# ORNL/HydraGNN

Hardware: NVIDIA H100
Metric: atoms_per_sec_training_step (higher is better)
Workload: dtype tf32

## Files before the change

### hydragnn_b200/csrc/hgb_painn_tc.cu

```cuda
#include "hgb_tc.cuh"

namespace {

enum { UPD_FWD, UPD_POST, UPD_BWD_A, UPD_BWD };

constexpr int UF = 64;
constexpr int UPD_TILE = 64;
constexpr uint32_t UPD_STAGE = UPD_TILE * UF * 4;
constexpr uint32_t UPD_B = 2 * UF * UF * 4;
constexpr uint32_t UPD_G = UPD_TILE * 2 * UF * 4;
constexpr int UPD_THREADS = 160;
constexpr int upd_stages(int mode) { return mode == UPD_BWD ? 5 : 4; }

struct UpdParams {
  int n;
  const float* wuv;
  const float* buv;
  const float* s;
  const float* a;
  const float* gs_out;
  const float* gv_out;
  const float* g_mlp_in;
  const float* mlp_in;
  float* mlp_in_out;
  float* inner_out;
  float* s_out;
  float* v_out;
  float* ga;
  float* g_uv;
  float* gs;
  float* gv;
};

constexpr size_t upd_smem(int mode) {
  return 1024 + (mode == UPD_BWD ? 2 : 1) * (size_t)UPD_B + upd_stages(mode) * (size_t)UPD_STAGE + (mode == UPD_BWD ? (size_t)UPD_G : 0) +
         2 * upd_stages(mode) * 8 + 2 * UF * 4;
}

__device__ __forceinline__ void frag_ld(float* x, const float* p, int64_t ld, int node, int n) {
#pragma unroll
  for (int h = 0; h < 2; ++h) {
    const bool in = node + 8 * h < n;
    const float* r = p + (int64_t)(node + 8 * h) * ld;
#pragma unroll
    for (int i = 0; i < 8; ++i) {
      const float2 t = in ? __ldg(reinterpret_cast<const float2*>(r + 8 * i)) : make_float2(0.f, 0.f);
      x[4 * i + 2 * h] = t.x;
      x[4 * i + 2 * h + 1] = t.y;
    }
  }
}
__device__ __forceinline__ void frag_st(float* p, int64_t ld, int node, int n, const float* x) {
#pragma unroll
  for (int h = 0; h < 2; ++h)
    if (node + 8 * h < n) {
      float* r = p + (int64_t)(node + 8 * h) * ld;
#pragma unroll
      for (int i = 0; i < 8; ++i) *reinterpret_cast<float2*>(r + 8 * i) = make_float2(x[4 * i + 2 * h], x[4 * i + 2 * h + 1]);
    }
}

__device__ __forceinline__ void prefetch_rows_l2(const float* base, int64_t ld, int row0, int rows, int col0, int cols) {
  if (cols == ld) {
    asm volatile("cp.async.bulk.prefetch.L2.global [%0], %1;" ::"l"(base + (int64_t)row0 * ld), "r"((uint32_t)(rows * ld * 4)) : "memory");
    return;
  }
  for (int r = 0; r < rows; ++r)
    asm volatile("cp.async.bulk.prefetch.L2.global [%0], %1;" ::"l"(base + (int64_t)(row0 + r) * ld + col0), "r"((uint32_t)(cols * 4))
                 : "memory");
}

}

template <int MODE, bool LAST>
__global__ void __launch_bounds__(UPD_THREADS, 1) painn_update_tc_kernel(const __grid_constant__ CUtensorMap tmap_v, const UpdParams p) {
  constexpr int NA = LAST ? 2 : 3;
  constexpr bool BWD = MODE == UPD_BWD;
  constexpr int S = upd_stages(MODE);
  extern __shared__ uint8_t smem_raw[];
  uint8_t* smem = reinterpret_cast<uint8_t*>((reinterpret_cast<uintptr_t>(smem_raw) + 1023) & ~(uintptr_t)1023);
  uint8_t* sB = smem;
  uint8_t* sBd = sB + UPD_B;
  uint8_t* sA = sBd + (BWD ? UPD_B : 0);
  uint8_t* sG = sA + S * UPD_STAGE;
  uint64_t* full = reinterpret_cast<uint64_t*>(sG + (BWD ? UPD_G : 0));
  uint64_t* empty = full + S;
  float* sbias = reinterpret_cast<float*>(empty + S);

  const int warp = threadIdx.x >> 5, lane = threadIdx.x & 31;
  const int ntiles = (p.n + UPD_TILE - 1) / UPD_TILE;
  for (int i = threadIdx.x; i < 2 * UF; i += blockDim.x) sbias[i] = __ldg(p.buv + i);
  if (threadIdx.x == 0) {
    for (int s = 0; s < S; ++s) { mbar_init(full + s, 1); mbar_init(empty + s, 4); }
    fence_barrier_init();
  }
  __syncthreads();

  if (warp == 4) {
    if (lane == 0) {
      uint32_t it = 0;
      for (int t = blockIdx.x; t < ntiles; t += gridDim.x) {
        const int row0 = t * UPD_TILE, rows = min(UPD_TILE, p.n - row0);
        if (MODE == UPD_FWD || MODE == UPD_POST) prefetch_rows_l2(p.s, UF, row0, rows, 0, UF);
        if (MODE == UPD_POST) prefetch_rows_l2(p.a, NA * UF, row0, rows, 0, NA * UF);
        if (MODE == UPD_BWD_A || BWD) prefetch_rows_l2(p.gs_out, UF, row0, rows, 0, UF);
        if ((MODE == UPD_BWD_A || BWD) && !LAST) prefetch_rows_l2(p.gv_out, 3 * UF, row0, rows, 0, 3 * UF);
        if (BWD) {
          prefetch_rows_l2(p.g_mlp_in, 2 * UF, row0, rows, 0, 2 * UF);
          prefetch_rows_l2(p.mlp_in, 2 * UF, row0, rows, 0, UF);
          prefetch_rows_l2(p.a, NA * UF, row0, rows, 0, (NA - 1) * UF);
        }
        for (int d = 0; d < 3; ++d, ++it) {
          const int s = it % S;
          mbar_wait(empty + s, ((it / S) & 1) ^ 1);
          mbar_expect_tx(full + s, UPD_STAGE);
          tma_load_3d(sA + (size_t)s * UPD_STAGE, &tmap_v, full + s, 0, d, t * UPD_TILE);
          tma_load_3d(sA + (size_t)s * UPD_STAGE + UPD_STAGE / 2, &tmap_v, full + s, 32, d, t * UPD_TILE);
        }
      }
    }
    return;
  }

  for (int i = threadIdx.x; i < 2 * UF * UF; i += 128) {
    const float w = __ldg(p.wuv + i);
    const int r = i / UF, c = i % UF;
    *reinterpret_cast<float*>(sB + kmajor_sw128_off(r, c, 2 * UF)) = w;
    if (BWD) *reinterpret_cast<float*>(sBd + kmajor_sw128_off(c, r, UF)) = w;
  }
  fence_proxy_async();
  named_bar_sync(1, 128);

  const int wq = warp;
  const int rsub = wq * 16 + (lane >> 2);
  const int c2 = 2 * (lane & 3);
  const uint32_t sA_addr = smem_u32(sA), sB_addr = smem_u32(sB), sBd_addr = smem_u32(sBd);
  const uint32_t sG_addr = smem_u32(sG);

  float acc[64];
  uint32_t it = 0;
  for (int t = blockIdx.x; t < ntiles; t += gridDim.x) {
    const int node = t * UPD_TILE + rsub;
    float x0[32], x1[32], x2[32];
    if (MODE == UPD_FWD) {
      frag_ld(x0, p.s + c2, UF, node, p.n);
      frag_st(p.mlp_in_out + UF + c2, 2 * UF, node, p.n, x0);
    }
    if ((MODE == UPD_POST || MODE == UPD_BWD) && !LAST) frag_ld(x2, p.a + c2, NA * UF, node, p.n);
    if (BWD) {
      float g[32], q[32];
      frag_ld(g, p.gs_out + c2, UF, node, p.n);
      frag_ld(q, p.g_mlp_in + UF + c2, 2 * UF, node, p.n);
#pragma unroll
      for (int j = 0; j < 32; ++j) q[j] = g[j] + q[j];
      frag_st(p.gs + c2, UF, node, p.n, q);
      frag_ld(x0, p.a + (NA - 2) * UF + c2, NA * UF, node, p.n);
#pragma unroll
      for (int j = 0; j < 32; ++j) x0[j] = g[j] * x0[j];
      frag_ld(x1, p.mlp_in + c2, 2 * UF, node, p.n);
      frag_ld(q, p.g_mlp_in + c2, 2 * UF, node, p.n);
#pragma unroll
      for (int j = 0; j < 32; ++j) {
        const float nrm = x1[j];
        x1[j] = nrm > 0.f ? q[j] / nrm : 0.f;
      }
    }
#pragma unroll 1
    for (int d = 0; d < 3; ++d, ++it) {
      const int s = it % S;
      float gvo[32];
// ... 68 lines not shown
          const int r = rsub + 8 * ((j >> 1) & 1), col = 8 * (j >> 2) + c2 + (j & 1);
          vo[j] = *reinterpret_cast<const float*>(st + kmajor_sw128_off(r, col, UPD_TILE)) + x2[j] * acc[j];
        }
        __syncwarp();
        if (lane == 0) mbar_arrive(empty + s);
        frag_st(p.v_out + d * UF + c2, 3 * UF, node, p.n, vo);
      }
      if (BWD) {
#pragma unroll
        for (int j = 0; j < 32; ++j) {
          const float u = acc[j], w = acc[32 + j];
          const float g_vo = LAST ? 0.f : gvo[j], a_vv = LAST ? 0.f : x2[j];
          acc[j] = fmaf(x0[j], w, g_vo * a_vv);
          acc[32 + j] = fmaf(x0[j], u, x1[j] * w);
        }
        frag_st(p.g_uv + d * 2 * UF + c2, 3 * 2 * UF, node, p.n, acc);
        frag_st(p.g_uv + d * 2 * UF + UF + c2, 3 * 2 * UF, node, p.n, acc + 32);
        named_bar_sync(1, 128);
#pragma unroll
        for (int j = 0; j < 32; j += 2) {
          const int r = rsub + 8 * ((j >> 1) & 1), col = 8 * (j >> 2) + c2;
          *reinterpret_cast<float2*>(sG + kmajor_sw128_off(r, col, UPD_TILE)) = make_float2(acc[j], acc[j + 1]);
          *reinterpret_cast<float2*>(sG + kmajor_sw128_off(r, UF + col, UPD_TILE)) = make_float2(acc[32 + j], acc[33 + j]);
        }
        fence_proxy_async();
        named_bar_sync(1, 128);
        float dg[32];
#pragma unroll
        for (int j = 0; j < 32; ++j) dg[j] = 0.f;
        fence_regs<32>(dg);
        wgmma_fence();
#pragma unroll
        for (int kb = 0; kb < 4; ++kb)
#pragma unroll
          for (int k4 = 0; k4 < 4; ++k4)
            wgmma_tf32<2>(dg, make_desc(sG_addr + kb * (UPD_G / 4) + k4 * 32), make_desc(sBd_addr + kb * UF * 128 + k4 * 32));
        wgmma_commit();
        wgmma_wait<0>();
        fence_regs<32>(dg);
#pragma unroll
        for (int j = 0; j < 32; ++j) {
          float y = dg[j] + 0.f;
          if (!LAST) y += gvo[j];
          dg[j] = y;
        }
        frag_st(p.gv + d * UF + c2, 3 * UF, node, p.n, dg);
      }
    }
    if (MODE == UPD_POST) {
      float sv[32], ss[32];
      frag_ld(x1, p.s + c2, UF, node, p.n);
      frag_ld(sv, p.a + (NA - 2) * UF + c2, NA * UF, node, p.n);
      frag_ld(ss, p.a + (NA - 1) * UF + c2, NA * UF, node, p.n);
#pragma unroll
      for (int j = 0; j < 32; ++j) x1[j] = x1[j] + sv[j] * x0[j] + ss[j];
      frag_st(p.s_out + c2, UF, node, p.n, x1);
    }
    if (MODE == UPD_BWD_A) {
      float g[32];
      frag_ld(g, p.gs_out + c2, UF, node, p.n);
      if (!LAST) frag_st(p.ga + c2, NA * UF, node, p.n, x1);
#pragma unroll
// ... 15 lines not shown
}
__global__ void painn_update_tc_bwd_a_last_kernel(const float* __restrict__ gs_out, const float* __restrict__ inner, int64_t nf,
                                                  float* __restrict__ ga) {
  for (int64_t t = (int64_t)blockIdx.x * blockDim.x + threadIdx.x; t < nf; t += (int64_t)gridDim.x * blockDim.x) {
    const int64_t i = t / UF;
    const int c = (int)(t % UF);
    const float g = gs_out[t];
    ga[i * 2 * UF + c] = g * inner[t];
    ga[i * 2 * UF + UF + c] = g;
  }
}

namespace {

template <int MODE, bool LAST>
int launch_update(const float* v, const UpdParams& p, hgb_stream_t stream, const char* name) {
  CUtensorMap tm;
  const cuuint64_t dims[3] = {(cuuint64_t)UF, 3, (cuuint64_t)p.n};
  const cuuint64_t strides[2] = {(cuuint64_t)UF * 4, (cuuint64_t)3 * UF * 4};
  const cuuint32_t box[3] = {32, 1, (cuuint32_t)UPD_TILE};
  int rc = encode_tmap(&tm, v, 3, dims, strides, box, CU_TENSOR_MAP_SWIZZLE_128B);
  if (rc) return rc;
  constexpr size_t smem = upd_smem(MODE);
  static_assert(smem <= SMEM_MAX, "painn_update_tc: shared memory budget");
  static int per_sm = 0;
  if (!per_sm) {
    cudaFuncSetAttribute(painn_update_tc_kernel<MODE, LAST>, cudaFuncAttributeMaxDynamicSharedMemorySize, (int)smem);
    if (cudaOccupancyMaxActiveBlocksPerMultiprocessor(&per_sm, painn_update_tc_kernel<MODE, LAST>, UPD_THREADS, smem) != cudaSuccess ||
        per_sm < 1)
      per_sm = 1;
  }
  const int ntiles = (p.n + UPD_TILE - 1) / UPD_TILE;
  const int grid = ntiles < per_sm * HGB_NUM_SMS ? ntiles : per_sm * HGB_NUM_SMS;
  painn_update_tc_kernel<MODE, LAST><<<grid, UPD_THREADS, smem, (cudaStream_t)stream>>>(tm, p);
  HGB_LAUNCH_CHECK(name);
  return HGB_OK;
}

bool al16(const void* q) { return ((uintptr_t)q & 15) == 0; }

UpdParams upd_params(int n, const float* wuv, const float* buv) {
  UpdParams p = {};
  p.n = n;
  p.wuv = wuv;
  p.buv = buv;
  return p;
}

}

// ... 36 lines not shown
  if (last) {
    const int64_t nf = (int64_t)n * UF;
    painn_update_tc_bwd_a_last_kernel<<<hgb_grid_for(nf, 256), 256, 0, (cudaStream_t)stream>>>(gs_out, inner, nf, ga);
    HGB_LAUNCH_CHECK("painn_update_tc_bwd_a_last");
    return HGB_OK;
  }
  UpdParams p = upd_params(n, wuv, buv);
  p.gs_out = gs_out;
  p.gv_out = gv_out;
  p.ga = ga;
  return launch_update<UPD_BWD_A, false>(v, p, stream, "painn_update_tc_bwd_a");
}

extern "C" int hgb_painn_update_tc_bwd(const float* v, const float* gs_out, const float* gv_out, const float* g_mlp_in, const float* a,
                                       const float* mlp_in, const float* wuv, const float* buv, int32_t n, int32_t last, float* g_uv,
                                       float* gs, float* gv, hgb_stream_t stream) {
  HGB_REQUIRE(n >= 0 && v && gs_out && g_mlp_in && a && mlp_in && wuv && buv && g_uv && gs && gv && (last || gv_out),
              "painn_update_tc_bwd: bad arguments");
  HGB_REQUIRE(al16(v) && al16(gs_out) && al16(g_mlp_in) && al16(a) && al16(mlp_in) && al16(g_uv) && al16(gs) && al16(gv) &&
                  (last || al16(gv_out)),
              "painn_update_tc_bwd: operands must be 16-byte aligned");
  if (n == 0) return HGB_OK;
  UpdParams p = upd_params(n, wuv, buv);
  p.gs_out = gs_out;
  p.gv_out = gv_out;
  p.g_mlp_in = g_mlp_in;
  p.a = a;
  p.mlp_in = mlp_in;
  p.g_uv = g_uv;
  p.gs = gs;
  p.gv = gv;
  return last ? launch_update<UPD_BWD, true>(v, p, stream, "painn_update_tc_bwd") : launch_update<UPD_BWD, false>(v, p, stream, "painn_update_tc_bwd");
}
```

### hydragnn_b200/csrc/hgb_tc.cu

```cuda
#include "hgb_tc.cuh"

namespace {

__device__ __forceinline__ void wgmma_n32(float* d, uint64_t ad, uint64_t bd) {
  asm volatile(
      "{\n"
      ".reg .pred p;\n"
      "setp.ne.b32 p, %18, 0;\n"
      "wgmma.mma_async.sync.aligned.m64n32k8.f32.tf32.tf32 "
      "{%0, %1, %2, %3, %4, %5, %6, %7, %8, %9, %10, %11, %12, %13, %14, %15}, %16, %17, p, 1, 1;\n"
      "}"
      : "+f"(d[0]), "+f"(d[1]), "+f"(d[2]), "+f"(d[3]), "+f"(d[4]), "+f"(d[5]), "+f"(d[6]), "+f"(d[7]), "+f"(d[8]), "+f"(d[9]),
        "+f"(d[10]), "+f"(d[11]), "+f"(d[12]), "+f"(d[13]), "+f"(d[14]), "+f"(d[15])
      : "l"(ad), "l"(bd), "r"(1));
}
__device__ __forceinline__ void wgmma_n16(float* d, uint64_t ad, uint64_t bd) {
  asm volatile(
      "{\n"
      ".reg .pred p;\n"
      "setp.ne.b32 p, %10, 0;\n"
      "wgmma.mma_async.sync.aligned.m64n16k8.f32.tf32.tf32 "
      "{%0, %1, %2, %3, %4, %5, %6, %7}, %8, %9, p, 1, 1;\n"
      "}"
      : "+f"(d[0]), "+f"(d[1]), "+f"(d[2]), "+f"(d[3]), "+f"(d[4]), "+f"(d[5]), "+f"(d[6]), "+f"(d[7])
      : "l"(ad), "l"(bd), "r"(1));
}

__device__ __forceinline__ float tf32_rna(float x) { return __uint_as_float((__float_as_uint(x) + 0x1000u) & 0xffffe000u); }

__device__ __forceinline__ void split_f4(const float4 v, float4& h, float4& l) {
  h.x = tf32_rna(v.x); h.y = tf32_rna(v.y); h.z = tf32_rna(v.z); h.w = tf32_rna(v.w);
  l.x = tf32_rna(v.x - h.x); l.y = tf32_rna(v.y - h.y); l.z = tf32_rna(v.z - h.z); l.w = tf32_rna(v.w - h.w);
}

struct LinParams {
  int m, kr, no;
  const float* w;
  int64_t ldw;
  int trans_b;
  const float* bias;
  int act;
// ... 576 lines not shown
  if (nc_max > 256) nc_max = 256;
  for (int c0 = 0; c0 < n_out; c0 += nc_max) {
    const int nc = n_out - c0 < nc_max ? n_out - c0 : nc_max;
    for (int k0 = 0; k0 < k_red; k0 += 256) {
      const int kc = k_red - k0 < 256 ? k_red - k0 : 256;
      const float* wp = trans_b ? w + (int64_t)k0 * ldw + c0 : w + (int64_t)c0 * ldw + k0;
      const float* add = k0 == 0 ? (addend ? addend + c0 : nullptr) : y + c0;
      int rc = tc_linear_piece(a + k0, lda, wp, ldw, trans_b, (bias && k0 == 0) ? bias + c0 : nullptr, m, nc, kc, act, act_param, y + c0,
                               z ? z + c0 : nullptr, add, gsrc ? gsrc + c0 : nullptr, gact, n_out, exact, stream);
      if (rc) return rc;
    }
  }
  return HGB_OK;
}

extern "C" int64_t hgb_tc_wgrad_workspace_bytes(int32_t n_out, int32_t k_out) { return (int64_t)HGB_NUM_SMS * n_out * (k_out + 1) * 4; }

extern "C" int hgb_tc_wgrad(const float* dz, int64_t lddz, const float* x, int64_t ldx, int32_t m, int32_t n_out, int32_t k_out,
                            float* dw, int64_t lddw, float* db, int32_t accumulate, int32_t exact, void* workspace,
                            int64_t workspace_bytes, hgb_stream_t stream) {
  HGB_REQUIRE(dz && x && dw && workspace && m >= 128 && shape_ok(k_out, n_out) && k_out + 16 <= 256,
              "tc_wgrad: unsupported shape m=%d n=%d k=%d", m, n_out, k_out);
  HGB_REQUIRE(lddz % 4 == 0 && ldx % 4 == 0 && ((uintptr_t)dz % 16 == 0) && ((uintptr_t)x % 16 == 0), "tc_wgrad: operands must be 16-byte aligned");
  HGB_REQUIRE(workspace_bytes >= hgb_tc_wgrad_workspace_bytes(n_out, k_out), "tc_wgrad: workspace too small");
  WgParams p;
  p.m = m; p.no = n_out; p.ko = k_out;
  p.split = exact ? 1 : 0;
  p.flush = exact ? 8 : 0;
  const int Q = k_out / 32;
  const int nsl_max = (n_out < WG_NA ? n_out : WG_NA) / 32;
// ... 5 lines not shown
  if (stages < 2) {
    tbufs = 1;
    stages = (int)((budget - tb_bytes) / raw_bytes);
  }
  if (stages > 4) stages = 4;
  HGB_REQUIRE(stages >= 2, "tc_wgrad: stage does not fit shared memory");
  p.stages = stages;
  p.tbufs = tbufs;
  CUtensorMap tdz, tx;
  int rc = make_tmap(&tdz, dz, m, n_out, lddz, WG_ROWS, CU_TENSOR_MAP_SWIZZLE_NONE);
  if (rc) return rc;
  rc = make_tmap(&tx, x, m, k_out, ldx, WG_ROWS, CU_TENSOR_MAP_SWIZZLE_NONE);
  if (rc) return rc;
  const int total_chunks = (m + WG_ROWS - 1) / WG_ROWS;
  const int gy = (n_out + WG_NA - 1) / WG_NA;
  const int max_x = HGB_NUM_SMS / gy;
  int gx = total_chunks < max_x ? total_chunks : max_x;
  p.chunks_per_cta = (total_chunks + gx - 1) / gx;
  gx = (total_chunks + p.chunks_per_cta - 1) / p.chunks_per_cta;
  p.part = (float*)workspace;
  const size_t smem = 1024 + tbufs * tb_bytes + stages * raw_bytes + 2 * stages * 8;
  cudaStream_t st = (cudaStream_t)stream;
  const dim3 grid(gx, gy);
  switch (Q) {
    case 1: launch_wgrad<1>(grid, smem, st, tdz, tx, p); break;
    case 2: launch_wgrad<2>(grid, smem, st, tdz, tx, p); break;
    case 3: launch_wgrad<3>(grid, smem, st, tdz, tx, p); break;
    case 4: launch_wgrad<4>(grid, smem, st, tdz, tx, p); break;
    case 5: launch_wgrad<5>(grid, smem, st, tdz, tx, p); break;
    case 6: launch_wgrad<6>(grid, smem, st, tdz, tx, p); break;
    default: launch_wgrad<7>(grid, smem, st, tdz, tx, p); break;
  }
  HGB_LAUNCH_CHECK("tc_wgrad");
  const int outs = n_out * (k_out + 1);
  tc_wgrad_reduce_kernel<<<(outs + 31) / 32, dim3(32, 8), 0, st>>>(p.part, gx, n_out, k_out, dw, lddw, db, accumulate);
  HGB_LAUNCH_CHECK("tc_wgrad_reduce");
  return HGB_OK;
}
```

### hydragnn_b200/csrc/hgb_tc.cuh

```cuda
#pragma once
#include <cuda.h>

#include "hgb_common.cuh"

namespace {

__device__ __forceinline__ uint32_t smem_u32(const void* p) { return (uint32_t)__cvta_generic_to_shared(p); }

__device__ __forceinline__ void mbar_init(uint64_t* bar, uint32_t count) {
  asm volatile("mbarrier.init.shared::cta.b64 [%0], %1;" ::"r"(smem_u32(bar)), "r"(count));
}
__device__ __forceinline__ void mbar_expect_tx(uint64_t* bar, uint32_t bytes) {
  asm volatile("mbarrier.arrive.expect_tx.shared::cta.b64 _, [%0], %1;" ::"r"(smem_u32(bar)), "r"(bytes) : "memory");
}
__device__ __forceinline__ void mbar_arrive(uint64_t* bar) {
  asm volatile("mbarrier.arrive.shared::cta.b64 _, [%0];" ::"r"(smem_u32(bar)) : "memory");
}
__device__ __forceinline__ void mbar_wait(uint64_t* bar, uint32_t parity) {
  asm volatile(
      "{\n"
      ".reg .pred P1;\n"
      "LAB_WAIT:\n"
      "mbarrier.try_wait.parity.shared::cta.b64 P1, [%0], %1;\n"
      "@P1 bra DONE;\n"
// ... 64 lines not shown
TC_WGMMA(2, "m64n64k8", "%32", "%33", "%34", TC_R16_0 ", " TC_R16_1, TC_D16(0), TC_D16(16))
TC_WGMMA(3, "m64n96k8", "%48", "%49", "%50", TC_R16_0 ", " TC_R16_1 ", " TC_R16_2, TC_D16(0), TC_D16(16), TC_D16(32))
TC_WGMMA(4, "m64n128k8", "%64", "%65", "%66", TC_R16_0 ", " TC_R16_1 ", " TC_R16_2 ", " TC_R16_3, TC_D16(0), TC_D16(16), TC_D16(32),
         TC_D16(48))
TC_WGMMA(5, "m64n160k8", "%80", "%81", "%82", TC_R16_0 ", " TC_R16_1 ", " TC_R16_2 ", " TC_R16_3 ", " TC_R16_4, TC_D16(0), TC_D16(16),
         TC_D16(32), TC_D16(48), TC_D16(64))
TC_WGMMA(6, "m64n192k8", "%96", "%97", "%98", TC_R16_0 ", " TC_R16_1 ", " TC_R16_2 ", " TC_R16_3 ", " TC_R16_4 ", " TC_R16_5, TC_D16(0),
         TC_D16(16), TC_D16(32), TC_D16(48), TC_D16(64), TC_D16(80))
TC_WGMMA(7, "m64n224k8", "%112", "%113", "%114", TC_R16_0 ", " TC_R16_1 ", " TC_R16_2 ", " TC_R16_3 ", " TC_R16_4 ", " TC_R16_5 ", " TC_R16_6,
         TC_D16(0), TC_D16(16), TC_D16(32), TC_D16(48), TC_D16(64), TC_D16(80), TC_D16(96))
TC_WGMMA(8, "m64n256k8", "%128", "%129", "%130", TC_R16_0 ", " TC_R16_1 ", " TC_R16_2 ", " TC_R16_3 ", " TC_R16_4 ", " TC_R16_5 ", " TC_R16_6
         ", " TC_R16_7, TC_D16(0), TC_D16(16), TC_D16(32), TC_D16(48), TC_D16(64), TC_D16(80), TC_D16(96), TC_D16(112))
#undef TC_WGMMA
#undef TC_D16

__device__ __forceinline__ void tma_store_2d(const CUtensorMap* tmap, const void* smem_src, int c0, int c1) {
  asm volatile("cp.async.bulk.tensor.2d.global.shared::cta.bulk_group [%0, {%2, %3}], [%1];" ::"l"(tmap), "r"(smem_u32(smem_src)),
               "r"(c0), "r"(c1)
               : "memory");
}
__device__ __forceinline__ void bulk_commit() { asm volatile("cp.async.bulk.commit_group;" ::: "memory"); }
template <int N>
__device__ __forceinline__ void bulk_wait_read() { asm volatile("cp.async.bulk.wait_group.read %0;" ::"n"(N) : "memory"); }
__device__ __forceinline__ void bulk_wait_all() { asm volatile("cp.async.bulk.wait_group 0;" ::: "memory"); }

__device__ __forceinline__ uint64_t make_desc(uint32_t saddr) {
  uint64_t d = 0;
  d |= (uint64_t)((saddr & 0x3FFFF) >> 4);
  d |= (uint64_t)1 << 16;
  d |= (uint64_t)(1024 >> 4) << 32;
// ... 35 lines not shown
  cuuint32_t estr[3] = {1, 1, 1};
  CUresult r = enc(tm, CU_TENSOR_MAP_DATA_TYPE_FLOAT32, rank, const_cast<float*>(base), dims, strides, box, estr, CU_TENSOR_MAP_INTERLEAVE_NONE,
                   swz, CU_TENSOR_MAP_L2_PROMOTION_L2_256B, CU_TENSOR_MAP_FLOAT_OOB_FILL_NONE);
  if (r != CUDA_SUCCESS) { hgb_set_error("tc: cuTensorMapEncodeTiled failed (%d)", (int)r); return HGB_ECUDA; }
  return HGB_OK;
}

int make_tmap(CUtensorMap* tm, const float* base, int64_t rows, int64_t cols, int64_t ld, int box_rows, CUtensorMapSwizzle swz) {
  const cuuint64_t gdim[2] = {(cuuint64_t)cols, (cuuint64_t)rows};
  const cuuint64_t gstr[1] = {(cuuint64_t)ld * 4};
  const cuuint32_t box[2] = {32, (cuuint32_t)box_rows};
  return encode_tmap(tm, base, 2, gdim, gstr, box, swz);
}

}
```

### hydragnn_b200/ops.py

```python
import os

import torch
from torch.autograd.function import once_differentiable

from . import _lib

ACT_CODES = {None: 0, "none": 0, "relu": 1, "silu": 2, "tanh": 3, "sigmoid": 4, "lrelu": 5, "elu": 6, "selu": 7}
POOL_CODES = {"add": 0, "sum": 0, "mean": 1, "max": 2}


def _stream():
    return torch.cuda.current_stream().cuda_stream


def _p(t):
    return None if t is None else t.data_ptr()


def _chk(t, dtype=torch.float32):
    if t is None:
        return None
    if not t.is_cuda:
        raise RuntimeError("hydragnn_b200 ops need CUDA tensors (no CPU fallback on the hot path)")
    if t.dtype != dtype:
# ... 862 lines not shown
    @staticmethod
    @once_differentiable
    def backward(ctx, gs_out, gv_out):
        v, mlp_in, z1, h, a, wuv, buv, w1, w2, inner = ctx.saved_tensors
        last = ctx.last
        n, f = mlp_in.shape[0], v.shape[2]
        gs_out = _aligned(gs_out)
        gv_out = None if last else _aligned(gv_out)
        ga = torch.empty_like(a)
        _lib.call("hgb_painn_update_tc_bwd_a", _p(v), _p(gs_out), _p(gv_out), _p(inner), _p(wuv), _p(buv), n, int(last), _p(ga), _stream())
        with tensor_cores(True):
            gz1, gw2, gb2 = linear_bwd_dispatch(ga, h, w2, dx_gsrc=z1, dx_gact=ctx.z1_code, leaves=ctx.leaves[2])
            g_mlp_in, gw1, gb1 = linear_bwd_dispatch(gz1, mlp_in, w1, leaves=ctx.leaves[1])
        g_uv = torch.empty(3 * n, 2 * f, dtype=v.dtype, device=v.device)
        gs, gv = torch.empty_like(gs_out), torch.empty_like(v)
        _lib.call("hgb_painn_update_tc_bwd", _p(v), _p(gs_out), _p(gv_out), _p(g_mlp_in), _p(a), _p(mlp_in), _p(wuv), _p(buv), n, int(last),
                  _p(g_uv), _p(gs), _p(gv), _stream())
        with tensor_cores(True):
            _, gwuv, gbuv = linear_bwd_dispatch(g_uv, v.reshape(3 * n, f), wuv, need_x=False, leaves=ctx.leaves[0])
        return gs, gv, gwuv[:f], gbuv[:f], gwuv[f:], gbuv[f:], gw1, gb1, gw2, gb2, None


SCALAR_UPDATE = os.environ.get("HGB_SCALAR", "1") == "1"


class PainnUpdateScalarFn(torch.autograd.Function):

    @staticmethod
    def forward(ctx, s, v, uw, ub, vw, vb, w1, b1, w2, b2, last):
        n = s.shape[0]
        na = 2 if last else 3
        pad = s.new_zeros(3 - na)
        pk = torch.cat([uw.reshape(1), ub.reshape(1), vw.reshape(1), vb.reshape(1), w1.reshape(2), b1.reshape(1), w2.reshape(na), pad,
                        b2.reshape(na), pad, s.new_zeros(3)]).contiguous()
# ... 586 lines not shown
```

### include/hgb.h

```cpp
#ifndef HGB_H
#define HGB_H

#include <stdint.h>

#ifdef __cplusplus
extern "C" {
#endif

typedef void* hgb_stream_t;

#define HGB_OK 0
#define HGB_EINVAL (-1)
#define HGB_ECUDA (-2)
#define HGB_ECAPACITY (-3)

#define HGB_ACT_DERIV 100
#define HGB_ACT_NONE 0
#define HGB_ACT_RELU 1
#define HGB_ACT_SILU 2
#define HGB_ACT_TANH 3
#define HGB_ACT_SIGMOID 4
#define HGB_ACT_LRELU 5
#define HGB_ACT_ELU 6
#define HGB_ACT_SELU 7
// ... 128 lines not shown
int hgb_painn_update_post_bwd_a(const float* gs_out, const float* gv_out, const float* uv,
                                const float* vv, int64_t ld, int32_t n, int32_t f, int32_t last, float* ga,
                                hgb_stream_t stream);
int hgb_painn_update_bwd(const float* gs_out, const float* gv_out, const float* g_mlp_in,
                         const float* a, const float* uv, const float* vv, int64_t ld, const float* mlp_in,
                         int32_t n, int32_t f, int32_t last, float* guv, float* gvv, float* gs,
                         float* gv, hgb_stream_t stream);
int hgb_painn_update_tc_fwd(const float* v, const float* s, const float* wuv, const float* buv, int32_t n,
                            float* mlp_in, float* inner, hgb_stream_t stream);
int hgb_painn_update_tc_post(const float* v, const float* s, const float* a, const float* inner, const float* wuv,
                             const float* buv, int32_t n, int32_t last, float* s_out, float* v_out, hgb_stream_t stream);
int hgb_painn_update_tc_bwd_a(const float* v, const float* gs_out, const float* gv_out, const float* inner,
                              const float* wuv, const float* buv, int32_t n, int32_t last, float* ga, hgb_stream_t stream);
int hgb_painn_update_tc_bwd(const float* v, const float* gs_out, const float* gv_out, const float* g_mlp_in,
                            const float* a, const float* mlp_in, const float* wuv, const float* buv, int32_t n,
                            int32_t last, float* g_uv, float* gs, float* gv, hgb_stream_t stream);


int hgb_mha_fwd(const float* qkv, int32_t n, int32_t f, int32_t heads, float* out, float* lse,
                hgb_stream_t stream);
int hgb_mha_bwd(const float* qkv, const float* out, const float* lse, const float* gout, int32_t n, int32_t f,
                int32_t heads, float* gqkv, hgb_stream_t stream);

int32_t hgb_mha_tc_supported(int32_t f, int32_t heads);
int hgb_mha_tc_fwd(const float* qkv, int32_t n, int32_t f, int32_t heads, int32_t exact, float* out, float* lse,
                   hgb_stream_t stream);
int hgb_mha_tc_bwd(const float* qkv, const float* out, const float* lse, const float* gout, int32_t n, int32_t f,
                   int32_t heads, int32_t exact, float* delta_ws, float* gqkv, hgb_stream_t stream);

int hgb_mace_tp_path(int32_t mode, const float* p0, const float* p1, const float* p2, const float* cg, int64_t e, int32_t f,
                     int32_t ni, int32_t nj, int32_t nk, float* out, hgb_stream_t stream);
// ... 104 lines not shown
```

Measured before the change: 41.76 million.

## Fuse PaiNN U/V weight-gradient GEMM into update backward kernel via warp specialization

```diff
diff --git a/hydragnn_b200/csrc/hgb_painn_tc.cu b/hydragnn_b200/csrc/hgb_painn_tc.cu
--- a/hydragnn_b200/csrc/hgb_painn_tc.cu
+++ b/hydragnn_b200/csrc/hgb_painn_tc.cu
@@ -9,8 +9,11 @@
 constexpr uint32_t UPD_STAGE = UPD_TILE * UF * 4;
 constexpr uint32_t UPD_B = 2 * UF * UF * 4;
 constexpr uint32_t UPD_G = UPD_TILE * 2 * UF * 4;
-constexpr int UPD_THREADS = 160;
-constexpr int upd_stages(int mode) { return mode == UPD_BWD ? 5 : 4; }
+constexpr uint32_t UPD_WT = (2 * UF + UF + 16) * 128;
+constexpr int UPD_STAGES = 4;
+constexpr int upd_threads(int mode) { return mode == UPD_BWD ? 384 : 160; }
+constexpr int UPD_PRODUCER_REGS = 40, UPD_CONSUMER_REGS = 256, UPD_WGRAD_REGS = 208;
+constexpr int BAR_WGRAD = 2;
 
 struct UpdParams {
   int n;
@@ -30,11 +33,15 @@
   float* g_uv;
   float* gs;
   float* gv;
+  float* part;
+  float* gwuv;
+  float* gbuv;
+  int chunks_per_cta;
 };
 
 constexpr size_t upd_smem(int mode) {
-  return 1024 + (mode == UPD_BWD ? 2 : 1) * (size_t)UPD_B + upd_stages(mode) * (size_t)UPD_STAGE + (mode == UPD_BWD ? (size_t)UPD_G : 0) +
-         2 * upd_stages(mode) * 8 + 2 * UF * 4;
+  return 1024 + (mode == UPD_BWD ? 2 : 1) * (size_t)UPD_B + UPD_STAGES * (size_t)UPD_STAGE +
+         (mode == UPD_BWD ? (size_t)UPD_G + 2 * UPD_WT + 16 : 0) + 2 * UPD_STAGES * 8 + 2 * UF * 4;
 }
 
 __device__ __forceinline__ void frag_ld(float* x, const float* p, int64_t ld, int node, int n) {
@@ -50,10 +57,10 @@
     }
   }
 }
-__device__ __forceinline__ void frag_st(float* p, int64_t ld, int node, int n, const float* x) {
+__device__ __forceinline__ void frag_st(float* p, int64_t ld, int node, int n, const float* x, int lo = 0) {
 #pragma unroll
   for (int h = 0; h < 2; ++h)
-    if (node + 8 * h < n) {
+    if (node + 8 * h < n && node + 8 * h >= lo) {
       float* r = p + (int64_t)(node + 8 * h) * ld;
 #pragma unroll
       for (int i = 0; i < 8; ++i) *reinterpret_cast<float2*>(r + 8 * i) = make_float2(x[4 * i + 2 * h], x[4 * i + 2 * h + 1]);
@@ -70,36 +77,136 @@
                  : "memory");
 }
 
+__device__ __forceinline__ uint32_t ld_acquire_shared(const uint32_t* q) {
+  uint32_t v;
+  asm volatile("ld.acquire.cta.shared::cta.u32 %0, [%1];" : "=r"(v) : "r"(smem_u32(q)) : "memory");
+  return v;
+}
+__device__ __forceinline__ void st_release_shared(uint32_t* q, uint32_t v) {
+  asm volatile("st.release.cta.shared::cta.u32 [%0], %1;" ::"r"(smem_u32(q)), "r"(v) : "memory");
+}
+
+__device__ __forceinline__ void upd_wgrad(const UpdParams& p, const float* v, uint8_t* tb, const uint32_t* tiles_done, int q_beg, int q_end,
+                                          int t_beg) {
+  constexpr int ROWS_T = 2 * UF + UF;
+  constexpr int ITEMS = ROWS_T * 8 / 128;
+  const int tq = threadIdx.x - 128, warp = threadIdx.x >> 5, lane = threadIdx.x & 31, wq = warp - 4;
+  const int rows = 3 * p.n;
+  float acc[2][2][16], accb[2][8];
+#pragma unroll
+  for (int m = 0; m < 2; ++m) {
+#pragma unroll
+    for (int j = 0; j < 16; ++j) acc[m][0][j] = acc[m][1][j] = 0.f;
+#pragma unroll
+    for (int j = 0; j < 8; ++j) accb[m][j] = 0.f;
+  }
+  for (int q = q_beg; q < q_end; ++q) {
+    const uint32_t need = (uint32_t)(q / 6 - t_beg + 1);
+    while (ld_acquire_shared(tiles_done) < need) __nanosleep(32);
+    float4 x[ITEMS];
+#pragma unroll
+    for (int k = 0; k < ITEMS; ++k) {
+      const int it = tq + 128 * k, r = it % ROWS_T, m4 = it / ROWS_T;
+      const float* src = r < 2 * UF ? p.g_uv + r : v + (r - 2 * UF);
+      const int ld = r < 2 * UF ? 2 * UF : UF, row = q * 32 + 4 * m4;
+      x[k].x = row < rows ? __ldcg(src + (int64_t)row * ld) : 0.f;
+      x[k].y = row + 1 < rows ? __ldcg(src + (int64_t)(row + 1) * ld) : 0.f;
+      x[k].z = row + 2 < rows ? __ldcg(src + (int64_t)(row + 2) * ld) : 0.f;
+      x[k].w = row + 3 < rows ? __ldcg(src + (int64_t)(row + 3) * ld) : 0.f;
+    }
+    uint8_t* t = tb + ((q - q_beg) & 1) * UPD_WT;
+    wgmma_wait<1>();
+    fence_regs<64>(&acc[0][0][0]);
+    fence_regs<16>(&accb[0][0]);
+    named_bar_sync(BAR_WGRAD, 128);
+#pragma unroll
+    for (int k = 0; k < ITEMS; ++k) {
+      const int it = tq + 128 * k, r = it % ROWS_T, m4 = it / ROWS_T;
+      *reinterpret_cast<float4*>(t + r * 128 + ((m4 ^ (r & 7)) << 4)) = x[k];
+    }
+    fence_proxy_async();
+    named_bar_sync(BAR_WGRAD, 128);
+    const uint32_t t_addr = smem_u32(t);
+    fence_regs<64>(&acc[0][0][0]);
+    fence_regs<16>(&accb[0][0]);
+    wgmma_fence();
+#pragma unroll
+    for (int k4 = 0; k4 < 4; ++k4)
+#pragma unroll
+      for (int m = 0; m < 2; ++m) {
+        const uint64_t ad = make_desc(t_addr + m * 64 * 128 + k4 * 32);
+#pragma unroll
+        for (int j = 0; j < 2; ++j) wgmma_n32(acc[m][j], ad, make_desc(t_addr + 2 * UF * 128 + j * 32 * 128 + k4 * 32));
+        wgmma_n16(accb[m], ad, make_desc(t_addr + ROWS_T * 128 + k4 * 32));
+      }
+    wgmma_commit();
+    fence_regs<64>(&acc[0][0][0]);
+    fence_regs<16>(&accb[0][0]);
+  }
+  wgmma_wait<0>();
+  fence_regs<64>(&acc[0][0][0]);
+  fence_regs<16>(&accb[0][0]);
+  float* part = p.part + (size_t)blockIdx.x * (2 * UF) * (UF + 1);
+#pragma unroll
+  for (int m = 0; m < 2; ++m)
+#pragma unroll
+    for (int h = 0; h < 2; ++h) {
+      float* pr = part + (size_t)(m * 64 + wq * 16 + (lane >> 2) + 8 * h) * (UF + 1);
+#pragma unroll
+      for (int j = 0; j < 2; ++j)
+#pragma unroll
+        for (int i = 0; i < 4; ++i)
+#pragma unroll
+          for (int e = 0; e < 2; ++e) pr[j * 32 + i * 8 + 2 * (lane & 3) + e] = acc[m][j][4 * i + 2 * h + e];
+      if ((lane & 3) == 0) pr[UF] = accb[m][2 * h];
+    }
+}
+
 }
 
 template <int MODE, bool LAST>
-__global__ void __launch_bounds__(UPD_THREADS, 1) painn_update_tc_kernel(const __grid_constant__ CUtensorMap tmap_v, const UpdParams p) {
+__global__ void __launch_bounds__(upd_threads(MODE), 1) painn_update_tc_kernel(const __grid_constant__ CUtensorMap tmap_v, const float* v_in,
+                                                                               const UpdParams p) {
   constexpr int NA = LAST ? 2 : 3;
   constexpr bool BWD = MODE == UPD_BWD;
-  constexpr int S = upd_stages(MODE);
+  constexpr int S = UPD_STAGES;
   extern __shared__ uint8_t smem_raw[];
   uint8_t* smem = reinterpret_cast<uint8_t*>((reinterpret_cast<uintptr_t>(smem_raw) + 1023) & ~(uintptr_t)1023);
   uint8_t* sB = smem;
   uint8_t* sBd = sB + UPD_B;
   uint8_t* sA = sBd + (BWD ? UPD_B : 0);
   uint8_t* sG = sA + S * UPD_STAGE;
-  uint64_t* full = reinterpret_cast<uint64_t*>(sG + (BWD ? UPD_G : 0));
+  uint8_t* sWT = sG + (BWD ? UPD_G : 0);
+  uint64_t* full = reinterpret_cast<uint64_t*>(sWT + (BWD ? 2 * UPD_WT : 0));
   uint64_t* empty = full + S;
-  float* sbias = reinterpret_cast<float*>(empty + S);
+  uint32_t* tiles_done = reinterpret_cast<uint32_t*>(empty + S);
+  float* sbias = reinterpret_cast<float*>(empty + S + (BWD ? 2 : 0));
 
   const int warp = threadIdx.x >> 5, lane = threadIdx.x & 31;
   const int ntiles = (p.n + UPD_TILE - 1) / UPD_TILE;
+  const int total_chunks = (3 * p.n + 31) / 32;
+  const int q_beg = blockIdx.x * p.chunks_per_cta, q_end = min(total_chunks, q_beg + p.chunks_per_cta);
+  const int r0 = q_beg * 32, r1 = min(q_end * 32, 3 * p.n);
+  const int t_beg = BWD ? r0 / (3 * UPD_TILE) : blockIdx.x;
+  const int t_end = BWD ? min(ntiles, (r1 + 3 * UPD_TILE - 1) / (3 * UPD_TILE)) : ntiles, t_step = BWD ? 1 : gridDim.x;
   for (int i = threadIdx.x; i < 2 * UF; i += blockDim.x) sbias[i] = __ldg(p.buv + i);
+  if (BWD) {
+    for (int i = threadIdx.x; i < 2 * 16 * 32; i += blockDim.x)
+      reinterpret_cast<float*>(sWT + (i >> 9) * UPD_WT + 3 * UF * 128)[i & 511] = 1.f;
+    fence_proxy_async();
+  }
   if (threadIdx.x == 0) {
     for (int s = 0; s < S; ++s) { mbar_init(full + s, 1); mbar_init(empty + s, 4); }
+    if (BWD) *tiles_done = 0;
     fence_barrier_init();
   }
   __syncthreads();
 
-  if (warp == 4) {
-    if (lane == 0) {
+  if (warp >= (BWD ? 8 : 4)) {
+    if constexpr (BWD) regs_dec<UPD_PRODUCER_REGS>();
+    if (warp == (BWD ? 8 : 4) && lane == 0) {
       uint32_t it = 0;
-      for (int t = blockIdx.x; t < ntiles; t += gridDim.x) {
+      for (int t = t_beg; t < t_end; t += t_step) {
         const int row0 = t * UPD_TILE, rows = min(UPD_TILE, p.n - row0);
         if (MODE == UPD_FWD || MODE == UPD_POST) prefetch_rows_l2(p.s, UF, row0, rows, 0, UF);
         if (MODE == UPD_POST) prefetch_rows_l2(p.a, NA * UF, row0, rows, 0, NA * UF);
@@ -121,6 +228,14 @@
     }
     return;
   }
+  if constexpr (BWD) {
+    if (warp >= 4) {
+      regs_inc<UPD_WGRAD_REGS>();
+      upd_wgrad(p, v_in, sWT, tiles_done, q_beg, q_end, t_beg);
+      return;
+    }
+    regs_inc<UPD_CONSUMER_REGS>();
+  }
 
   for (int i = threadIdx.x; i < 2 * UF * UF; i += 128) {
     const float w = __ldg(p.wuv + i);
@@ -139,8 +254,9 @@
 
   float acc[64];
   uint32_t it = 0;
-  for (int t = blockIdx.x; t < ntiles; t += gridDim.x) {
+  for (int t = t_beg; t < t_end; t += t_step) {
     const int node = t * UPD_TILE + rsub;
+    const int n_own = !BWD || t * 3 * UPD_TILE >= r0 ? p.n : 0;
     float x0[32], x1[32], x2[32];
     if (MODE == UPD_FWD) {
       frag_ld(x0, p.s + c2, UF, node, p.n);
@@ -153,7 +269,7 @@
       frag_ld(q, p.g_mlp_in + UF + c2, 2 * UF, node, p.n);
 #pragma unroll
       for (int j = 0; j < 32; ++j) q[j] = g[j] + q[j];
-      frag_st(p.gs + c2, UF, node, p.n, q);
+      frag_st(p.gs + c2, UF, node, n_own, q);
       frag_ld(x0, p.a + (NA - 2) * UF + c2, NA * UF, node, p.n);
 #pragma unroll
       for (int j = 0; j < 32; ++j) x0[j] = g[j] * x0[j];
@@ -252,8 +368,8 @@
           acc[j] = fmaf(x0[j], w, g_vo * a_vv);
           acc[32 + j] = fmaf(x0[j], u, x1[j] * w);
         }
-        frag_st(p.g_uv + d * 2 * UF + c2, 3 * 2 * UF, node, p.n, acc);
-        frag_st(p.g_uv + d * 2 * UF + UF + c2, 3 * 2 * UF, node, p.n, acc + 32);
+        frag_st(p.g_uv + d * 2 * UF + c2, 3 * 2 * UF, node, min(p.n, (r1 - d + 2) / 3), acc, (r0 - d + 2) / 3);
+        frag_st(p.g_uv + d * 2 * UF + UF + c2, 3 * 2 * UF, node, min(p.n, (r1 - d + 2) / 3), acc + 32, (r0 - d + 2) / 3);
         named_bar_sync(1, 128);
 #pragma unroll
         for (int j = 0; j < 32; j += 2) {
@@ -282,8 +398,12 @@
           if (!LAST) y += gvo[j];
           dg[j] = y;
         }
-        frag_st(p.gv + d * UF + c2, 3 * UF, node, p.n, dg);
-      }
+        frag_st(p.gv + d * UF + c2, 3 * UF, node, n_own, dg);
+      }
+    }
+    if (BWD) {
+      named_bar_sync(1, 128);
+      if (threadIdx.x == 0) st_release_shared(tiles_done, (uint32_t)(t - t_beg + 1));
     }
     if (MODE == UPD_POST) {
       float sv[32], ss[32];
@@ -329,7 +449,7 @@
 namespace {
 
 template <int MODE, bool LAST>
-int launch_update(const float* v, const UpdParams& p, hgb_stream_t stream, const char* name) {
+int launch_update(const float* v, UpdParams p, hgb_stream_t stream, const char* name) {
   CUtensorMap tm;
   const cuuint64_t dims[3] = {(cuuint64_t)UF, 3, (cuuint64_t)p.n};
   const cuuint64_t strides[2] = {(cuuint64_t)UF * 4, (cuuint64_t)3 * UF * 4};
@@ -338,17 +458,25 @@
   if (rc) return rc;
   constexpr size_t smem = upd_smem(MODE);
   static_assert(smem <= SMEM_MAX, "painn_update_tc: shared memory budget");
+  constexpr int threads = upd_threads(MODE);
   static int per_sm = 0;
   if (!per_sm) {
     cudaFuncSetAttribute(painn_update_tc_kernel<MODE, LAST>, cudaFuncAttributeMaxDynamicSharedMemorySize, (int)smem);
-    if (cudaOccupancyMaxActiveBlocksPerMultiprocessor(&per_sm, painn_update_tc_kernel<MODE, LAST>, UPD_THREADS, smem) != cudaSuccess ||
+    if (cudaOccupancyMaxActiveBlocksPerMultiprocessor(&per_sm, painn_update_tc_kernel<MODE, LAST>, threads, smem) != cudaSuccess ||
         per_sm < 1)
       per_sm = 1;
   }
   const int ntiles = (p.n + UPD_TILE - 1) / UPD_TILE;
-  const int grid = ntiles < per_sm * HGB_NUM_SMS ? ntiles : per_sm * HGB_NUM_SMS;
-  painn_update_tc_kernel<MODE, LAST><<<grid, UPD_THREADS, smem, (cudaStream_t)stream>>>(tm, p);
+  int grid = ntiles < per_sm * HGB_NUM_SMS ? ntiles : per_sm * HGB_NUM_SMS;
+  if (MODE == UPD_BWD) {
+    static_assert(MODE != UPD_BWD || 2 * smem > SMEM_MAX, "painn_update_tc: BWD runs one CTA per SM");
+    const int total_chunks = (3 * p.n + 31) / 32;
+    p.chunks_per_cta = wgrad_chunks_per_cta(total_chunks, HGB_NUM_SMS);
+    grid = (total_chunks + p.chunks_per_cta - 1) / p.chunks_per_cta;
+  }
+  painn_update_tc_kernel<MODE, LAST><<<grid, threads, smem, (cudaStream_t)stream>>>(tm, v, p);
   HGB_LAUNCH_CHECK(name);
+  if (MODE == UPD_BWD) return tc_wgrad_reduce(p.part, grid, 2 * UF, UF, p.gwuv, UF, p.gbuv, 0, (cudaStream_t)stream);
   return HGB_OK;
 }
 
@@ -415,13 +543,21 @@
 
 extern "C" int hgb_painn_update_tc_bwd(const float* v, const float* gs_out, const float* gv_out, const float* g_mlp_in, const float* a,
                                        const float* mlp_in, const float* wuv, const float* buv, int32_t n, int32_t last, float* g_uv,
-                                       float* gs, float* gv, hgb_stream_t stream) {
-  HGB_REQUIRE(n >= 0 && v && gs_out && g_mlp_in && a && mlp_in && wuv && buv && g_uv && gs && gv && (last || gv_out),
+                                       float* gs, float* gv, float* gwuv, float* gbuv, void* workspace, int64_t workspace_bytes,
+                                       hgb_stream_t stream) {
+  HGB_REQUIRE(n >= 0 && n <= (1 << 29) && v && gs_out && g_mlp_in && a && mlp_in && wuv && buv && g_uv && gs && gv && gwuv && gbuv &&
+                  workspace && (last || gv_out),
               "painn_update_tc_bwd: bad arguments");
   HGB_REQUIRE(al16(v) && al16(gs_out) && al16(g_mlp_in) && al16(a) && al16(mlp_in) && al16(g_uv) && al16(gs) && al16(gv) &&
-                  (last || al16(gv_out)),
+                  al16(workspace) && (last || al16(gv_out)),
               "painn_update_tc_bwd: operands must be 16-byte aligned");
-  if (n == 0) return HGB_OK;
+  HGB_REQUIRE(workspace_bytes >= hgb_tc_wgrad_workspace_bytes(2 * UF, UF), "painn_update_tc_bwd: workspace too small");
+  if (n == 0) {
+    HGB_REQUIRE(cudaMemsetAsync(gwuv, 0, 2 * UF * UF * sizeof(float), (cudaStream_t)stream) == cudaSuccess &&
+                    cudaMemsetAsync(gbuv, 0, 2 * UF * sizeof(float), (cudaStream_t)stream) == cudaSuccess,
+                "painn_update_tc_bwd: zeroing the weight gradient failed");
+    return HGB_OK;
+  }
   UpdParams p = upd_params(n, wuv, buv);
   p.gs_out = gs_out;
   p.gv_out = gv_out;
@@ -431,5 +567,8 @@
   p.g_uv = g_uv;
   p.gs = gs;
   p.gv = gv;
+  p.part = static_cast<float*>(workspace);
+  p.gwuv = gwuv;
+  p.gbuv = gbuv;
   return last ? launch_update<UPD_BWD, true>(v, p, stream, "painn_update_tc_bwd") : launch_update<UPD_BWD, false>(v, p, stream, "painn_update_tc_bwd");
 }
diff --git a/hydragnn_b200/csrc/hgb_tc.cu b/hydragnn_b200/csrc/hgb_tc.cu
--- a/hydragnn_b200/csrc/hgb_tc.cu
+++ b/hydragnn_b200/csrc/hgb_tc.cu
@@ -1,30 +1,6 @@
 #include "hgb_tc.cuh"
 
 namespace {
-
-__device__ __forceinline__ void wgmma_n32(float* d, uint64_t ad, uint64_t bd) {
-  asm volatile(
-      "{\n"
-      ".reg .pred p;\n"
-      "setp.ne.b32 p, %18, 0;\n"
-      "wgmma.mma_async.sync.aligned.m64n32k8.f32.tf32.tf32 "
-      "{%0, %1, %2, %3, %4, %5, %6, %7, %8, %9, %10, %11, %12, %13, %14, %15}, %16, %17, p, 1, 1;\n"
-      "}"
-      : "+f"(d[0]), "+f"(d[1]), "+f"(d[2]), "+f"(d[3]), "+f"(d[4]), "+f"(d[5]), "+f"(d[6]), "+f"(d[7]), "+f"(d[8]), "+f"(d[9]),
-        "+f"(d[10]), "+f"(d[11]), "+f"(d[12]), "+f"(d[13]), "+f"(d[14]), "+f"(d[15])
-      : "l"(ad), "l"(bd), "r"(1));
-}
-__device__ __forceinline__ void wgmma_n16(float* d, uint64_t ad, uint64_t bd) {
-  asm volatile(
-      "{\n"
-      ".reg .pred p;\n"
-      "setp.ne.b32 p, %10, 0;\n"
-      "wgmma.mma_async.sync.aligned.m64n16k8.f32.tf32.tf32 "
-      "{%0, %1, %2, %3, %4, %5, %6, %7}, %8, %9, p, 1, 1;\n"
-      "}"
-      : "+f"(d[0]), "+f"(d[1]), "+f"(d[2]), "+f"(d[3]), "+f"(d[4]), "+f"(d[5]), "+f"(d[6]), "+f"(d[7])
-      : "l"(ad), "l"(bd), "r"(1));
-}
 
 __device__ __forceinline__ float tf32_rna(float x) { return __uint_as_float((__float_as_uint(x) + 0x1000u) & 0xffffe000u); }
 
@@ -631,6 +607,13 @@
   return HGB_OK;
 }
 
+int tc_wgrad_reduce(const float* part, int nparts, int no, int ko, float* dw, int64_t lddw, float* db, int accumulate, cudaStream_t st) {
+  const int outs = no * (ko + 1);
+  tc_wgrad_reduce_kernel<<<(outs + 31) / 32, dim3(32, 8), 0, st>>>(part, nparts, no, ko, dw, lddw, db, accumulate);
+  HGB_LAUNCH_CHECK("tc_wgrad_reduce");
+  return HGB_OK;
+}
+
 extern "C" int64_t hgb_tc_wgrad_workspace_bytes(int32_t n_out, int32_t k_out) { return (int64_t)HGB_NUM_SMS * n_out * (k_out + 1) * 4; }
 
 extern "C" int hgb_tc_wgrad(const float* dz, int64_t lddz, const float* x, int64_t ldx, int32_t m, int32_t n_out, int32_t k_out,
@@ -666,10 +649,8 @@
   if (rc) return rc;
   const int total_chunks = (m + WG_ROWS - 1) / WG_ROWS;
   const int gy = (n_out + WG_NA - 1) / WG_NA;
-  const int max_x = HGB_NUM_SMS / gy;
-  int gx = total_chunks < max_x ? total_chunks : max_x;
-  p.chunks_per_cta = (total_chunks + gx - 1) / gx;
-  gx = (total_chunks + p.chunks_per_cta - 1) / p.chunks_per_cta;
+  p.chunks_per_cta = wgrad_chunks_per_cta(total_chunks, HGB_NUM_SMS / gy);
+  const int gx = (total_chunks + p.chunks_per_cta - 1) / p.chunks_per_cta;
   p.part = (float*)workspace;
   const size_t smem = 1024 + tbufs * tb_bytes + stages * raw_bytes + 2 * stages * 8;
   cudaStream_t st = (cudaStream_t)stream;
@@ -684,8 +665,5 @@
     default: launch_wgrad<7>(grid, smem, st, tdz, tx, p); break;
   }
   HGB_LAUNCH_CHECK("tc_wgrad");
-  const int outs = n_out * (k_out + 1);
-  tc_wgrad_reduce_kernel<<<(outs + 31) / 32, dim3(32, 8), 0, st>>>(p.part, gx, n_out, k_out, dw, lddw, db, accumulate);
-  HGB_LAUNCH_CHECK("tc_wgrad_reduce");
-  return HGB_OK;
-}
+  return tc_wgrad_reduce(p.part, gx, n_out, k_out, dw, lddw, db, accumulate, st);
+}
diff --git a/hydragnn_b200/csrc/hgb_tc.cuh b/hydragnn_b200/csrc/hgb_tc.cuh
--- a/hydragnn_b200/csrc/hgb_tc.cuh
+++ b/hydragnn_b200/csrc/hgb_tc.cuh
@@ -102,6 +102,35 @@
 #undef TC_WGMMA
 #undef TC_D16
 
+__device__ __forceinline__ void wgmma_n32(float* d, uint64_t ad, uint64_t bd) {
+  asm volatile(
+      "{\n"
+      ".reg .pred p;\n"
+      "setp.ne.b32 p, %18, 0;\n"
+      "wgmma.mma_async.sync.aligned.m64n32k8.f32.tf32.tf32 "
+      "{%0, %1, %2, %3, %4, %5, %6, %7, %8, %9, %10, %11, %12, %13, %14, %15}, %16, %17, p, 1, 1;\n"
+      "}"
+      : "+f"(d[0]), "+f"(d[1]), "+f"(d[2]), "+f"(d[3]), "+f"(d[4]), "+f"(d[5]), "+f"(d[6]), "+f"(d[7]), "+f"(d[8]), "+f"(d[9]),
+        "+f"(d[10]), "+f"(d[11]), "+f"(d[12]), "+f"(d[13]), "+f"(d[14]), "+f"(d[15])
+      : "l"(ad), "l"(bd), "r"(1));
+}
+__device__ __forceinline__ void wgmma_n16(float* d, uint64_t ad, uint64_t bd) {
+  asm volatile(
+      "{\n"
+      ".reg .pred p;\n"
+      "setp.ne.b32 p, %10, 0;\n"
+      "wgmma.mma_async.sync.aligned.m64n16k8.f32.tf32.tf32 "
+      "{%0, %1, %2, %3, %4, %5, %6, %7}, %8, %9, p, 1, 1;\n"
+      "}"
+      : "+f"(d[0]), "+f"(d[1]), "+f"(d[2]), "+f"(d[3]), "+f"(d[4]), "+f"(d[5]), "+f"(d[6]), "+f"(d[7])
+      : "l"(ad), "l"(bd), "r"(1));
+}
+
+inline int wgrad_chunks_per_cta(int total_chunks, int max_ctas) {
+  const int ctas = total_chunks < max_ctas ? total_chunks : max_ctas;
+  return (total_chunks + ctas - 1) / ctas;
+}
+
 __device__ __forceinline__ void tma_store_2d(const CUtensorMap* tmap, const void* smem_src, int c0, int c1) {
   asm volatile("cp.async.bulk.tensor.2d.global.shared::cta.bulk_group [%0, {%2, %3}], [%1];" ::"l"(tmap), "r"(smem_u32(smem_src)),
                "r"(c0), "r"(c1)
@@ -167,3 +196,5 @@
 }
 
 }
+
+int tc_wgrad_reduce(const float* part, int nparts, int no, int ko, float* dw, int64_t lddw, float* db, int accumulate, cudaStream_t st);
diff --git a/hydragnn_b200/ops.py b/hydragnn_b200/ops.py
--- a/hydragnn_b200/ops.py
+++ b/hydragnn_b200/ops.py
@@ -900,10 +900,11 @@
             g_mlp_in, gw1, gb1 = linear_bwd_dispatch(gz1, mlp_in, w1, leaves=ctx.leaves[1])
         g_uv = torch.empty(3 * n, 2 * f, dtype=v.dtype, device=v.device)
         gs, gv = torch.empty_like(gs_out), torch.empty_like(v)
+        gwuv, gbuv = torch.empty_like(wuv), torch.empty_like(buv)
+        nbytes = _lib.query("hgb_tc_wgrad_workspace_bytes", 2 * f, f)
+        ws = _ws(nbytes, v.device)
         _lib.call("hgb_painn_update_tc_bwd", _p(v), _p(gs_out), _p(gv_out), _p(g_mlp_in), _p(a), _p(mlp_in), _p(wuv), _p(buv), n, int(last),
-                  _p(g_uv), _p(gs), _p(gv), _stream())
-        with tensor_cores(True):
-            _, gwuv, gbuv = linear_bwd_dispatch(g_uv, v.reshape(3 * n, f), wuv, need_x=False, leaves=ctx.leaves[0])
+                  _p(g_uv), _p(gs), _p(gv), _p(gwuv), _p(gbuv), _p(ws), nbytes, _stream())
         return gs, gv, gwuv[:f], gbuv[:f], gwuv[f:], gbuv[f:], gw1, gb1, gw2, gb2, None
 
 
diff --git a/include/hgb.h b/include/hgb.h
--- a/include/hgb.h
+++ b/include/hgb.h
@@ -166,7 +166,8 @@
                               const float* wuv, const float* buv, int32_t n, int32_t last, float* ga, hgb_stream_t stream);
 int hgb_painn_update_tc_bwd(const float* v, const float* gs_out, const float* gv_out, const float* g_mlp_in,
                             const float* a, const float* mlp_in, const float* wuv, const float* buv, int32_t n,
-                            int32_t last, float* g_uv, float* gs, float* gv, hgb_stream_t stream);
+                            int32_t last, float* g_uv, float* gs, float* gv, float* gwuv, float* gbuv,
+                            void* workspace, int64_t workspace_bytes, hgb_stream_t stream);
 
 
 int hgb_mha_fwd(const float* qkv, int32_t n, int32_t f, int32_t heads, float* out, float* lse,
diff --git a/profiles/painn_uv_wgrad.py b/profiles/painn_uv_wgrad.py
--- /dev/null
+++ b/profiles/painn_uv_wgrad.py
@@ -0,0 +1,64 @@
+import json
+import os
+import sys
+sys.path.insert(0, os.path.dirname(os.path.dirname(os.path.abspath(__file__))))
+import torch
+from hydragnn_b200 import _lib, ops
+from hydragnn_b200.stacks import PainnUpdate
+
+dev = torch.device("cuda")
+flush = torch.empty(256 * 1024 * 1024, dtype=torch.uint8, device=dev)
+
+
+def timeit(fn, iters=20, warm=3):
+    ts = []
+    for it in range(iters + warm):
+        flush.zero_()
+        a, b = torch.cuda.Event(enable_timing=True), torch.cuda.Event(enable_timing=True)
+        a.record(); fn(); b.record(); torch.cuda.synchronize()
+        if it >= warm:
+            ts.append(a.elapsed_time(b))
+    ts.sort()
+    return round(ts[len(ts) // 2] * 1e3, 1)
+
+
+n = int(sys.argv[1]) if len(sys.argv) > 1 else 147456
+f = 64
+g = torch.Generator(device=dev).manual_seed(0)
+r = lambda *s: torch.randn(*s, device=dev, generator=g)
+v, gs_out, gv_out, g_mlp_in = r(n, 3, f), r(n, f), r(n, 3, f), r(n, 2 * f)
+a, mlp_in = r(n, 3 * f), r(n, 2 * f).abs()
+wuv, buv = r(2 * f, f) * 0.1, r(2 * f) * 0.1
+g_uv, gs, gv = torch.empty(3 * n, 2 * f, device=dev), torch.empty_like(gs_out), torch.empty_like(v)
+out = {"n": n}
+gw, gb = torch.empty(2 * f, f, device=dev), torch.empty(2 * f, device=dev)
+nbytes = _lib.query("hgb_tc_wgrad_workspace_bytes", 2 * f, f)
+ws = ops._ws(nbytes, dev)
+for last in (True, False):
+    go = None if last else gv_out
+    call = lambda: _lib.call("hgb_painn_update_tc_bwd", ops._p(v), ops._p(gs_out), ops._p(go), ops._p(g_mlp_in), ops._p(a),
+                             ops._p(mlp_in), ops._p(wuv), ops._p(buv), n, int(last), ops._p(g_uv), ops._p(gs), ops._p(gv), ops._p(gw),
+                             ops._p(gb), ops._p(ws), nbytes, ops._stream())
+    out["update_tc_bwd (+ U/V weight gradient) last=%s (us)" % last] = timeit(call)
+
+dz, x2 = r(3 * n, 2 * f), v.reshape(3 * n, f)
+with ops.tensor_cores(True):
+    out["tc_wgrad m=%d n=128 k=64 (us)" % (3 * n)] = timeit(lambda: ops.raw_tc_wgrad(dz, x2))
+
+overlap = ops.WGRAD_OVERLAP
+ops.WGRAD_OVERLAP = False
+try:
+    for last in (True, False):
+        upd = PainnUpdate(f, last).to(dev)
+        params = [upd.update_U.weight, upd.update_U.bias, upd.update_V.weight, upd.update_V.bias, upd.update_mlp[0].weight,
+                  upd.update_mlp[0].bias, upd.update_mlp[2].weight, upd.update_mlp[2].bias]
+        s, vv = r(n, f).requires_grad_(True), v.clone().requires_grad_(True)
+        with ops.tensor_cores(True):
+            so, vo = ops.PainnUpdateTcFn.apply(s, vv, *params, last)
+            outs = (so,) if last else (so, vo)
+            grads = tuple(torch.randn_like(o) for o in outs)
+            out["PainnUpdateTcFn backward last=%s (us)" % last] = timeit(
+                lambda: torch.autograd.grad(outs, [s, vv] + params, grads, retain_graph=True))
+finally:
+    ops.WGRAD_OVERLAP = overlap
+print(json.dumps(out, indent=1))
```

Result: slower. 41.15 million (median of 6 runs) (-1.5%).
